# HiKapok/DAN

Hardware: AMD Instinct MI355X
Metric: 640x640 images/sec/node (train fwd+bwd) (higher is better)
Workload: dtype bf16; 1 GPU; S3FD VGG-16 backbone + 6 detection heads, 640x640 bf16 training (fwd+bwd+SGD), batch 16 per GPU; global_batch=16, parallelism=dp1, anchors_per_image=34125, step_launch=eager, rccl_ranks=1, weight_gradient_stream=True

## Files before the change

### dan_amd/_lib.py

```python
import ctypes
import os

import torch

_HERE = os.path.dirname(os.path.abspath(__file__))
ACT_NAME = os.environ.get("DANHIP_DTYPE", "bf16").lower()
if ACT_NAME not in ("bf16", "fp16"):
    raise ValueError("DANHIP_DTYPE must be bf16 or fp16, got %r" % ACT_NAME)
ACT_DTYPE = torch.float16 if ACT_NAME == "fp16" else torch.bfloat16
SO_PATH = os.path.join(_HERE, "libdanhip_f16.so" if ACT_NAME == "fp16" else "libdanhip.so")
if os.environ.get("DANHIP_LIB_PATH"):
    SO_PATH = os.path.abspath(os.environ["DANHIP_LIB_PATH"])

F32, BF16 = 0, 1
SPLIT3 = 3


class ConvDesc(ctypes.Structure):
    _fields_ = [(n, ctypes.c_int32) for n in ("N", "H", "W", "Cin", "Ho", "Wo", "Cout", "kh", "kw", "stride")]


class ConvPitch(ctypes.Structure):
    _fields_ = [(n, ctypes.c_int32) for n in ("x_pitch", "y_pitch", "aux_pitch")]


class PackEntry(ctypes.Structure):
    _fields_ = [("w_hwio", ctypes.c_void_p), ("wf_packed", ctypes.c_void_p), ("wb_packed", ctypes.c_void_p)] + \
               [(n, ctypes.c_int32) for n in ("kh", "kw", "cin", "cin_real", "cout", "rows_f", "cols_f", "rows_b", "cols_b", "co8", "first_block", "pad_")]


HEADS_MAX_LEVELS = 8


class HeadLevel(ctypes.Structure):
    _fields_ = [("h", ctypes.c_void_p), ("dy", ctypes.c_void_p)] + [(n, ctypes.c_int32) for n in ("HW", "Ch", "nneg", "npos", "off", "co_pad")]


class JpegInfo(ctypes.Structure):
    _fields_ = [(n, ctypes.c_int32) for n in ("width", "height", "ncomp", "mode", "reason", "reserved")] + [("coef_count", ctypes.c_int64)]


class JpegDesc(ctypes.Structure):
    _fields_ = [(n, ctypes.c_int32) for n in ("width", "height", "ncomp", "mode")] + \
               [(n, ctypes.c_int32 * 3) for n in ("blocks_w", "blocks_h", "comp_w", "comp_h", "quant_index")] + \
               [(n, ctypes.c_int32) for n in ("status", "idct_groups", "rgb_groups")] + [("reserved", ctypes.c_int32 * 2)] + \
               [("coef_offset", ctypes.c_int64), ("coef_count", ctypes.c_int64), ("plane_offset", ctypes.c_int64 * 3),
                ("out_offset", ctypes.c_int64), ("quant", (ctypes.c_uint16 * 64) * 4)]


P = ctypes.c_void_p
I32 = ctypes.c_int32
I64 = ctypes.c_int64
FL = ctypes.c_float
DESC = ctypes.POINTER(ConvDesc)

SIGNATURES = {
    "danhip_conv_packed_dims": [DESC, ctypes.c_int, ctypes.POINTER(I64), ctypes.POINTER(I64)],
    "danhip_pack_conv_weight": [DESC, P, I32, P, P, P],
    "danhip_conv2d_fwd_pool": [DESC, P, P, P, P, P, P],
    "danhip_pack_entry_init": [ctypes.POINTER(PackEntry), DESC, P, I32, P, P, I32, ctypes.POINTER(ctypes.c_int32)],
    "danhip_pack_conv_weights_batched": [P, I32, I32, P],
    "danhip_conv2d_fwd": [DESC, P, P, P, P, ctypes.c_int, ctypes.c_int, P, P],
    "danhip_conv2d_fwd_ws": [DESC, P, P, P, P, ctypes.c_int, ctypes.c_int, P, P, ctypes.c_size_t, P],
    "danhip_conv2d_fwd_f32": [DESC, P, P, P, P, ctypes.c_int, P, P],
# ... 54 lines not shown
    "danhip_dynamic_anchor_routing_eval": [P, P, P, P, I64, I32, I32, I32, I32, I32, P, P, P, ctypes.c_size_t, P],
    "danhip_dynamic_anchor_routing_train": [P, P, P, P, I64, I32, I32, I32, I32, I32, FL, FL, ctypes.c_uint64, ctypes.c_uint64, P, P, P, P,
                                            ctypes.c_size_t, P],
    "danhip_nms": [P, I32, I32, I32, FL, P, P, P],
    "danhip_argsort_desc_f32": [P, I64, I32, P, P, ctypes.c_size_t, P],
    "danhip_augment_preprocess": [P, I32, I32, I32, ctypes.POINTER(ctypes.c_int32), ctypes.POINTER(ctypes.c_float), I32, I32, I32, I32, I32, P, I32, I32,
                                  P, ctypes.c_size_t, P],
    "danhip_deform_psroi_pool_fwd": [P, P, P, P, P, I32, I32, I32, I32, I32, I32, I32, I32, I32, FL, FL, I32, I32, P],
    "danhip_deform_psroi_pool_bwd": [P, P, P, P, P, P, P, I32, I32, I32, I32, I32, I32, I32, I32, I32, I32, FL, FL, I32, I32, P],
    "danhip_maxpool3x3s2_same_fwd": [P, P, I32, I32, I32, I32, P],
    "danhip_maxpool3x3s2_same_bwd": [P, P, P, I32, I32, I32, I32, P],
    "danhip_resize_u8_linear": [P, I32, I32, P, I32, I32, I32, ctypes.c_double, ctypes.c_double, P],
    "danhip_bbox_vote": [P, P, I32, I32, ctypes.c_double, I32, P, P, P, ctypes.c_size_t, P],
    "danhip_wider_quantize": [P, ctypes.c_int, P, P, I32, I32, I32, P, P, I32, I32, P, P],
    "danhip_wider_score_range": [P, I64, P, P, ctypes.c_size_t, P],
    "danhip_wider_eval": [P, P, I64, P, P, P, I64, P, I32, I32, I32, I32, ctypes.c_double, P, ctypes.c_size_t, P, P],
    "danhip_wider_ap": [P, ctypes.c_size_t, P, I64, I32, I32, I32, P, P, P, P, P, P],
    "danhip_deform_sample_fwd": [P, P, P, I32, I32, I32, I32, I32, I32, I32, I32, I32, P],
    "danhip_deform_sample_bwd": [P, P, P, P, P, I32, I32, I32, I32, I32, I32, I32, I32, I32, ctypes.c_int, P, ctypes.c_size_t, P],
    "danhip_deform_conv_fwd": [P, P, P, P, P, I32, I32, I32, I32, I32, I32, I32, I32, I32, I32, ctypes.c_int, P, ctypes.c_size_t, P],
    "danhip_deform_conv_bwd": [P, P, P, P, P, P, P, P, I32, I32, I32, I32, I32, I32, I32, I32, I32, I32, ctypes.c_int, P, ctypes.c_size_t, P],
    "danhip_deform_conv_bwd_with_col": [P, P, P, P, P, P, P, P, P, I32, I32, I32, I32, I32, I32, I32, I32, I32, I32, ctypes.c_int, P, ctypes.c_size_t, P],
    "danhip_deform_conv_bwd_deliver": [P, P, P, P, P, P, P, P, P, I32, I32, I32, I32, I32, I32, I32, I32, I32, I32, ctypes.c_int, ctypes.c_int, P, ctypes.c_size_t, P],
    "danhip_cast_pad_f32_to_bf16": [P, P, P, I64, I32, I32, P],
    "danhip_head_split_fwd": [P, P, P, I32, I32, I32, I32, I32, I32, I32, P],
    "danhip_head_split_bwd": [P, P, P, P, I32, I32, I32, I32, I32, I32, I32, P],
    "danhip_heads_split_fwd": [ctypes.POINTER(HeadLevel), I32, P, P, I32, I32, P],
    "danhip_heads_grad_pad": [ctypes.POINTER(HeadLevel), I32, P, P, I32, I32, P],
    "danhip_hard_neg_select": [P, P, P, P, P, P, I32, I32, FL, ctypes.c_int, P],
    "danhip_detection_loss_fwd": [P, P, P, P, P, P, P, P, I32, I32, P],
    "danhip_detection_loss_bwd": [P, P, P, P, P, P, P, FL, FL, I32, I32, P],
    "danhip_sgd_momentum_flat": [P, P, P, P, P, P, I32, I64, FL, FL, FL, P, P],
    "danhip_sgd_momentum_flat_dynamic": [P, P, P, P, P, P, I32, I64, FL, FL, P, P, P],
    "danhip_anchors_generate": [P, P, P, P, P, P, I32, I32, I32, FL, FL, FL, I32, P],
    "danhip_iou_matrix": [P, P, P, P, P, P, P, I32, I32, P],
    "danhip_dual_max_match": [P, I32, I32, FL, FL, ctypes.c_int, P, P, P, ctypes.c_size_t, P],
    "danhip_small_mining_match": [P, I32, I32, FL, FL, FL, I32, FL, P, P, P, ctypes.c_size_t, P],
    "danhip_encode_anchors": [P, P, P, P, P, P, P, P, P, I32, FL, FL, FL, FL, FL, P],
    "danhip_decode_anchors": [P, P, P, P, P, P, I32, I32, FL, FL, FL, FL, P],
    "danhip_face_scores": [P, P, P, FL, I64, P],
    "danhip_comm_load": [ctypes.c_char_p],
    "danhip_comm_rccl_version": [ctypes.POINTER(ctypes.c_int)],
    "danhip_comm_unique_id": [P],
    "danhip_comm_create": [P, I32, I32, I32, ctypes.POINTER(ctypes.c_void_p)],
    "danhip_comm_destroy": [P],
    "danhip_comm_info": [P, ctypes.POINTER(I32), ctypes.POINTER(I32), ctypes.POINTER(I32)],
    "danhip_comm_async_error": [P, ctypes.POINTER(I32)],
    "danhip_comm_abort": [P],
    "danhip_comm_allreduce_sum": [P, P, I64, ctypes.c_int, P],
    "danhip_comm_reduce_scatter_sum": [P, P, P, I64, ctypes.c_int, P],
    "danhip_comm_allgather": [P, P, P, I64, ctypes.c_int, P],
    "danhip_jpeg_entropy_decode_batch": [P, P, I32, I32, P, I64, P, P],
    "danhip_jpeg_entropy_decode_batch_ex": [P, P, I32, I32, ctypes.c_uint32, P, I64, P, P],
    "danhip_jpeg_scan_prepare_batch_ex": [P, P, I32, ctypes.c_uint32, P, ctypes.c_size_t, I64, P, P],
    "danhip_jpeg_reconstruct_batch": [P, I64, P, P, I32, P, I64, P, ctypes.c_size_t, P, P],
    "danhip_jpeg_scan_prepare_batch": [P, P, I32, P, ctypes.c_size_t, I64, P, P],
    "danhip_jpeg_huffman_decode_batch": [P, P, ctypes.c_size_t, I32, P, I64, P, P, P, ctypes.c_size_t, P, P, P],
    "danhip_jpeg_entropy_emulate_batch": [P, ctypes.c_size_t, I32, P, P, I64, I32, P, P],
    "danhip_encode_anchors_batched": [P] * 11 + [I32, I32, I32, I32, I32, FL, FL, FL, I32, FL, FL, FL, FL, FL, FL, P, P, P, P, P,
                                                 ctypes.c_size_t, P],
}

_lib = None


class DanhipError(RuntimeError):
# ... 128 lines not shown
```

### dan_amd/csrc/capi.cpp

```cpp
#include <cstdarg>
#include <cstdio>
#include <cstdlib>
#include <cstring>
#include <atomic>
#include <mutex>

#include <hip/hip_runtime.h>

#include "../../include/danhip.h"

static thread_local char g_err[512] = "";

void danhip_set_error(const char* fmt, ...) {
  va_list ap;
  va_start(ap, fmt);
  vsnprintf(g_err, sizeof(g_err), fmt, ap);
  va_end(ap);
}

extern "C" const char* danhip_last_error(void) { return g_err; }
extern "C" int danhip_version(void) { return 10; }
extern "C" int danhip_act_dtype(void) {
#ifdef DANHIP_FP16
  return DANHIP_F16;
#else
  return DANHIP_BF16;
#endif
}

namespace {
struct Opt { const char* name; const char* env; int def; std::atomic<int> value; };
Opt g_opts[] = {{"splitk", "DANHIP_SPLITK", 1, {0}}, {"wgrad_slab", "DANHIP_WGRAD_SLAB", 1, {0}}, {"halo_b2", "DANHIP_HALO_B2", 0, {0}},
                {"wgrad_b2", "DANHIP_WGRAD_B2", 0, {0}}, {"halo_general_epilogue", "DANHIP_HALO_GENERAL_EPILOGUE", 0, {0}},
                {"deform_bwd_form", "DANHIP_DEFORM_BWD_FORM", 0, {0}}, {"pw_dgrad_ld_bn", "DANHIP_PW_DGRAD_LD_BN", 128, {0}},
                {"wgrad_c8", "DANHIP_WGRAD_C8", 1, {0}}, {"deform_dx_untiled", "DANHIP_DEFORM_DX_UNTILED", 0, {0}},
                {"deterministic", "DANHIP_DETERMINISTIC", 0, {0}}};
std::once_flag g_opts_once;
Opt* find_opt(const char* name) {
  std::call_once(g_opts_once, [] {
    for (Opt& o : g_opts) { const char* e = getenv(o.env); o.value.store(e ? atoi(e) : o.def, std::memory_order_relaxed); }
  });
  if (!name) return nullptr;
  for (Opt& o : g_opts)
    if (strcmp(o.name, name) == 0) return &o;
  return nullptr;
}
}

int danhip_option(const char* name) {
  Opt* o = find_opt(name);
  return o ? o->value.load(std::memory_order_relaxed) : 0;
}
extern "C" int danhip_get_option(const char* name) { return danhip_option(name); }

// ... 16 lines not shown
```

### dan_amd/csrc/loss.hip

```cpp
#include "common.h"

namespace {

__device__ __forceinline__ float block_sum(float v, float* sh) {
#pragma unroll
  for (int o = 32; o > 0; o >>= 1) v += __shfl_xor(v, o, 64);
  const int w = threadIdx.x >> 6, nw = blockDim.x >> 6;
  if ((threadIdx.x & 63) == 0) sh[w] = v;
  __syncthreads();
  float t = 0.f;
  for (int i = 0; i < nw; ++i) t += sh[i];
  __syncthreads();
  return t;
}

__global__ void head_split_fwd_kernel(const float* __restrict__ h, float* __restrict__ loc, float* __restrict__ cls, int B, int HW, int Ch,
                                      int nneg, int npos, int A, int off) {
  const long total = (long)B * HW;
  for (long m = (long)blockIdx.x * blockDim.x + threadIdx.x; m < total; m += (long)gridDim.x * blockDim.x) {
    const int b = (int)(m / HW), p = (int)(m % HW);
    const float* r = h + m * Ch;
    const long a = (long)b * A + off + p;
    *reinterpret_cast<float4*>(loc + a * 4) = make_float4(r[0], r[1], r[2], r[3]);
    float ng = r[4];
    for (int i = 1; i < nneg; ++i) ng = fmaxf(ng, r[4 + i]);
    float ps = r[4 + nneg];
    for (int i = 1; i < npos; ++i) ps = fmaxf(ps, r[4 + nneg + i]);
    *reinterpret_cast<float2*>(cls + a * 2) = make_float2(ng, ps);
  }
}

__global__ void head_split_bwd_kernel(const float* __restrict__ h, const float* __restrict__ dloc, const float* __restrict__ dcls,
                                      float* __restrict__ dy, int B, int HW, int Ch, int nneg, int npos, int A, int off) {
// ... 267 lines not shown
    float4 d = make_float4(0.f, 0.f, 0.f, 0.f);
    if (s == 2) {
      const float4 p = *reinterpret_cast<const float4*>(loc + i * 4);
      const float4 t = *reinterpret_cast<const float4*>(loc_t + i * 4);
      const float df[4] = {p.x - t.x, p.y - t.y, p.z - t.z, p.w - t.w};
      float o[4];
#pragma unroll
      for (int j = 0; j < 4; ++j) o[j] = (fabsf(df[j]) < 1.f ? df[j] : (df[j] > 0.f ? 1.f : -1.f)) * kl;
      d = make_float4(o[0], o[1], o[2], o[3]);
    }
    *reinterpret_cast<float4*>(dloc + i * 4) = d;
  }
}

__global__ void sgd_momentum_flat_kernel(float* __restrict__ w, const float* __restrict__ g, float* __restrict__ v, const long* __restrict__ seg,
                                         const float* __restrict__ gmult, const float* __restrict__ wdc, int nseg, long total, float lr,
                                         float momentum, float gscale, float* __restrict__ l2_out, const float* __restrict__ dyn,
                                         float* __restrict__ l2_part) {
  __shared__ float sh[8];
  float l2 = 0.f;
  bool skip = false;
  if (dyn) { gscale = 1.f / dyn[0]; skip = dyn[3] != 0.f; }
  const long n4 = total >> 2;
  const long stride = (long)gridDim.x * blockDim.x;
  long q = (long)blockIdx.x * blockDim.x + threadIdx.x;
  int lo = 0;
  if (q < n4) {
    int hi = nseg;
    while (hi - lo > 1) { const int mid = (lo + hi) >> 1; if (seg[mid] <= q * 4) lo = mid; else hi = mid; }
  }
  auto update = [&](long qq, int sg, float4 wi, const float4 gi, float4 vi) __attribute__((always_inline)) {
    const float c = wdc[sg], gm = gmult[sg];
    l2 += 0.5f * c * (wi.x * wi.x + wi.y * wi.y + wi.z * wi.z + wi.w * wi.w);
    vi.x = momentum * vi.x + (gi.x * gscale + c * wi.x) * gm;
    vi.y = momentum * vi.y + (gi.y * gscale + c * wi.y) * gm;
    vi.z = momentum * vi.z + (gi.z * gscale + c * wi.z) * gm;
    vi.w = momentum * vi.w + (gi.w * gscale + c * wi.w) * gm;
    wi.x -= lr * vi.x; wi.y -= lr * vi.y; wi.z -= lr * vi.z; wi.w -= lr * vi.w;
    if (!skip) {
      reinterpret_cast<float4*>(v)[qq] = vi;
      reinterpret_cast<float4*>(w)[qq] = wi;
    }
  };
  for (; q + stride < n4; q += 2 * stride) {
    const long q1 = q + stride;
    const float4 w0 = reinterpret_cast<const float4*>(w)[q], w1 = reinterpret_cast<const float4*>(w)[q1];
    const float4 g0 = reinterpret_cast<const float4*>(g)[q], g1 = reinterpret_cast<const float4*>(g)[q1];
    const float4 v0 = reinterpret_cast<const float4*>(v)[q], v1 = reinterpret_cast<const float4*>(v)[q1];
    while (lo + 1 < nseg && seg[lo + 1] <= q * 4) ++lo;
    int lo1 = lo;
    while (lo1 + 1 < nseg && seg[lo1 + 1] <= q1 * 4) ++lo1;
    update(q, lo, w0, g0, v0);
    update(q1, lo1, w1, g1, v1);
    lo = lo1;
  }
  for (; q < n4; q += stride) {
    while (lo + 1 < nseg && seg[lo + 1] <= q * 4) ++lo;
    update(q, lo, reinterpret_cast<const float4*>(w)[q], reinterpret_cast<const float4*>(g)[q], reinterpret_cast<const float4*>(v)[q]);
  }
  if (l2_out) {
    l2 = block_sum(l2, sh);
    if (threadIdx.x == 0) {
      if (l2_part) l2_part[blockIdx.x] = l2;
      else atomicAdd(l2_out, l2);
    }
  }
}

__global__ void grad_nonfinite_kernel(const float* __restrict__ g, long total, float* __restrict__ dyn) {
  bool bad = false;
  const long n4 = total >> 2;
// ... 225 lines not shown
```

### dan_amd/ops.py

```python
import contextlib
import ctypes
import os

import torch

from . import _lib
from ._lib import ACT_DTYPE as ACT, BF16, F32, SPLIT3, ConvDesc, call, ptr, stream


class OpsContext(object):
    __slots__ = ("USE_SPLITK", "USE_SLOTS", "USE_RELU_BITS", "USE_POOL_ARG", "USE_JUNCTION", "POOL_ONLY_TRAIN", "KEEP_DEFORM_COL", "WGRAD_STREAM", "WGRAD_FIRST", "FUSE_FIRST_WGRAD", "HEADS_BATCHED", "SPLIT_EVAL", "deterministic", "TRACE",
                 "PROFILE", "PROFILE_BYTES", "GRAD_READY_HOOK", "LOSS_SCALE_DEV", "wgrad")

    def __init__(self, **overrides):
        env = os.environ.get
        self.USE_SPLITK = True
        self.USE_SLOTS = True
        self.USE_RELU_BITS = env("DANHIP_RELU_BITS", "1") == "1"
        self.USE_POOL_ARG = env("DANHIP_POOL_ARG", "1") == "1"
        self.USE_JUNCTION = env("DANHIP_JUNCTION", "1") == "1"
        self.POOL_ONLY_TRAIN = env("DANHIP_POOL_ONLY_TRAIN", "1") == "1"
        self.KEEP_DEFORM_COL = True
        self.WGRAD_STREAM = env("DANHIP_WGRAD_STREAM", "1") == "1"
        self.WGRAD_FIRST = env("DANHIP_WGRAD_FIRST", "0") == "1"
        self.FUSE_FIRST_WGRAD = env("DANHIP_FUSE_FIRST_WGRAD", "1") == "1"
        self.HEADS_BATCHED = env("DANHIP_HEADS_BATCHED", "1") == "1"
        self.SPLIT_EVAL = False
        self.deterministic = env("DANHIP_DETERMINISTIC", "0") == "1"
        self.TRACE = self.PROFILE = self.PROFILE_BYTES = None
        self.GRAD_READY_HOOK = self.LOSS_SCALE_DEV = None
        self.wgrad = {"on": False, "side": None, "main": None, "keep": []}
        for k, v in overrides.items():
            setattr(self, k, v)


_CTX = OpsContext()
_CTX_FIELDS = frozenset(OpsContext.__slots__) - {"wgrad"}


def context():
    return _CTX


@contextlib.contextmanager
def use_context(ctx):
    global _CTX
    prev, _CTX = _CTX, ctx
    _sync_deterministic(prev, ctx)
    try:
        yield ctx
    finally:
        _CTX = prev
        _sync_deterministic(ctx, prev)


def _sync_deterministic(old, new):
    if bool(old.deterministic) != bool(new.deterministic):
        call("danhip_set_option", b"deterministic", 1 if new.deterministic else 0)

# ... 74 lines not shown
    st = _stamp(w_param)
    if e.stamp != st:
        wd = w_param.detach()
        if not (wd.dtype == torch.float32 and wd.is_contiguous()):
            raise RuntimeError("packed_weights: a kernel variable of shape %s arrives as a non-contiguous view (strides %s): it is a member of a "
                               "fused parameter block, which only the fused op consumes - set the fused / unfused switches BEFORE the "
                               "trainer (FlatParams) is built, not between calls" % (tuple(wd.shape), tuple(wd.stride())))
        call("danhip_pack_conv_weight", ctypes.byref(e.d), ptr(wd), wd.shape[2], ptr(e.wf), ptr(e.wb), stream())
        e.stamp = st
    return e.wf, (e.wb if need_bwd else None)


def repack_all(key=None, select=None):
    entries = [(e, e.ref()) for e in _PACKED.values()]
    entries = [(e, p) for e, p in entries if p is not None and (select is None or select(p))]
    if not entries:
        return
    tabs = _PACK_TABLE_OF
    tab = tabs.get(key)
    ids, ptrs = [id(p) for _, p in entries], [p.data_ptr() for _, p in entries]
    if tab is None or tab[3] != ids or tab[4] != ptrs:
        arr = (_lib.PackEntry * len(entries))()
        first = 0
        nb = ctypes.c_int32()
        for i, (e, p) in enumerate(entries):
            call("danhip_pack_entry_init", ctypes.byref(arr[i]), ctypes.byref(e.d), ptr(p.detach()), p.shape[2], ptr(e.wf), ptr(e.wb), first,
                 ctypes.byref(nb))
            first += nb.value
        host = torch.frombuffer(bytearray(bytes(arr)), dtype=torch.uint8)
        tab = tabs[key] = (len(entries), host.to(entries[0][1].device), first, ids, ptrs)
    n, dev_tab, blocks, _, _ = tab
    call("danhip_pack_conv_weights_batched", ptr(dev_tab), n, blocks, stream())
    for e, p in entries:
        e.stamp = _stamp(p)


def _grad_sink(p):
    return getattr(p, "_danhip_grad", None)


def _sink_trainable(t):
    ms = getattr(t, "_danhip_members", None)
    return ms is not None and any(m.requires_grad for m in ms)


def _prof_begin(st=None):
    if _CTX.PROFILE is None:
        return None
    e = torch.cuda.Event(enable_timing=True)
    e.record(st if st is not None else torch.cuda.current_stream())
    return e


def _prof_end(e0, d, which, st=None, wrote_y=True, pooled=False):
    if e0 is None:
        return
    e1 = torch.cuda.Event(enable_timing=True)
    e1.record(st if st is not None else torch.cuda.current_stream())
    if which == 2:
        label = _lib.lib().danhip_conv_wgrad_kernel_label(ctypes.byref(d)).decode()
    else:
        label = _lib.lib().danhip_conv_kernel_label(ctypes.byref(d), which).decode()
    cin = d.Cin
    flops = 2.0 * d.N * d.Ho * d.Wo * cin * d.Cout * d.kh * d.kw
    _CTX.PROFILE.setdefault(label, []).append((e0, e1, flops))
    if _CTX.PROFILE_BYTES is not None:
# ... 1603 lines not shown
```

### dan_amd/trainer.py

```python
import atexit
import ctypes
import os
import sys
import weakref

import torch
import torch.distributed as dist

from ._lib import call, ptr, stream


def comm_timeout_s():
    return float(os.environ.get("DANHIP_COMM_TIMEOUT_S", "300"))


DEADLINE_EXIT_CODE = 75


def _die(msg):
    sys.stderr.write("dan_amd: FATAL (rank %s): %s\n" % (os.environ.get("RANK", "0"), msg))
    sys.stderr.flush()
    os._exit(DEADLINE_EXIT_CODE)


# ... 374 lines not shown
            self.g.index_fill_(0, self.struct_zero_idx, 0.0)

    def range_plan(self, s, e):
        k0, k1 = self.starts.index(s), (self.starts.index(e) if e < self.total else len(self.starts))
        rel = (self.seg[k0:k1 + 1] - s).contiguous()
        idx = None
        if self.struct_zero_idx is not None:
            m = (self.struct_zero_idx >= s) & (self.struct_zero_idx < e)
            idx = self.struct_zero_idx[m].contiguous() if bool(m.any()) else None
        return k0, k1 - k0, rel, idx

    def sgd_range(self, s, e, plan, lr, momentum=0.9, grad_scale=1.0):
        k0, nseg, rel, idx = plan
        if idx is not None:
            self.g.index_fill_(0, idx, 0.0)
        off = ctypes.c_void_p
        base = lambda t, elems: off(t.data_ptr() + 4 * elems)
        call("danhip_sgd_momentum_flat", base(self.w, s), base(self.g, s), base(self.v, s), ptr(rel), base(self.gmult, k0), base(self.wdc, k0), nseg,
             e - s, float(lr), float(momentum), float(grad_scale), ptr(self.l2), stream())

    def sgd_step(self, lr, momentum=0.9, grad_scale=1.0, dynamic_state=None, deterministic=False):
        self.mask_structured()
        self.l2.zero_()
        if dynamic_state is not None:
            call("danhip_sgd_momentum_flat_dynamic", ptr(self.w), ptr(self.g), ptr(self.v), ptr(self.seg), ptr(self.gmult), ptr(self.wdc),
                 len(self.names), self.total, float(lr), float(momentum), ptr(dynamic_state), ptr(self.l2), stream())
        elif deterministic:
            if getattr(self, "_sgd_ws", None) is None:
                from . import _lib
                self._sgd_ws = torch.empty(int(_lib.lib().danhip_sgd_workspace_bytes()), dtype=torch.uint8, device=self.w.device)
            call("danhip_sgd_momentum_flat_ws", ptr(self.w), ptr(self.g), ptr(self.v), ptr(self.seg), ptr(self.gmult), ptr(self.wdc), len(self.names),
                 self.total, float(lr), float(momentum), float(grad_scale), ptr(self.l2), ptr(self._sgd_ws), self._sgd_ws.numel(), stream())
        else:
            call("danhip_sgd_momentum_flat", ptr(self.w), ptr(self.g), ptr(self.v), ptr(self.seg), ptr(self.gmult), ptr(self.wdc), len(self.names),
                 self.total, float(lr), float(momentum), float(grad_scale), ptr(self.l2), stream())
        from . import ops
        ops.WEIGHT_EPOCH += 1
        ops.repack_all()


class GradBuckets(object):

    def __init__(self, flat, bucket_bytes=32 << 20, tail_bytes=2 << 20):
        self.flat = flat
        self.on_bucket = None
        self.local = False
        self.enabled = (dist.is_available() and dist.is_initialized() and dist.get_world_size() > 1) or (os.environ.get("DANHIP_FORCE_DIST") == "1" and flat.g.is_cuda)
        self.fake = (not self.enabled) and os.environ.get("DANHIP_FAKE_ALLREDUCE") == "1" and flat.g.is_cuda
        self.enabled = self.enabled or self.fake
        self.bucket_bytes = bucket_bytes
        per = max(1, bucket_bytes // 4)
        self.bounds = []
        end = flat.total
        cur_end = end
        for s in reversed(flat.starts):
            if cur_end - s >= per:
                self.bounds.append((s, cur_end))
                cur_end = s
        if cur_end > 0:
            self.bounds.append((0, cur_end))
        s0, e0 = self.bounds[-1]
        tail = max(1, tail_bytes // 4)
        if e0 - s0 > 2 * tail:
            cut = max((st for st in flat.starts if s0 < st <= s0 + tail), default=None)
            if cut is not None and cut < e0:
                self.bounds[-1:] = [(cut, e0), (s0, cut)]
# ... 181 lines not shown
```

### include/danhip.h

```cpp
#ifndef DANHIP_H_
#define DANHIP_H_
#include <stddef.h>
#include <stdint.h>

#ifdef __cplusplus
extern "C" {
#endif

#define DANHIP_OK 0
#define DANHIP_EINVAL (-1)
#define DANHIP_ELAUNCH (-2)
#define DANHIP_EWORKSPACE (-3)

#define DANHIP_F32 0
#define DANHIP_BF16 1
#define DANHIP_F16 2
#define DANHIP_SPLIT3 3

const char* danhip_last_error(void);
int danhip_version(void);
int danhip_set_option(const char* name, int value);
int danhip_get_option(const char* name);
int danhip_act_dtype(void);

// ... 129 lines not shown
int danhip_head_split_bwd(const float* h, const float* dloc, const float* dcls, float* dy, int32_t B, int32_t HW, int32_t Ch,
                          int32_t nneg, int32_t npos, int32_t A, int32_t anchor_offset, void* stream);
#define DANHIP_HEADS_MAX_LEVELS 8
typedef struct danhip_head_level {
  const float* h;
  uint16_t* dy;
  int32_t HW, Ch, nneg, npos;
  int32_t off;
  int32_t co_pad;
} danhip_head_level;
int danhip_heads_split_fwd(const danhip_head_level* levels, int32_t nlevels, float* loc, float* cls, int32_t B, int32_t A, void* stream);
int danhip_heads_grad_pad(const danhip_head_level* levels, int32_t nlevels, const float* dloc, const float* dcls, int32_t B, int32_t A,
                          void* stream);
int danhip_hard_neg_select(const float* cls, const int32_t* labels, float* score, int32_t* counts, float* thr, int32_t* k_out,
                           int32_t B, int32_t A, float negative_ratio, int at_least_one, void* stream);
int danhip_detection_loss_fwd(const float* cls, const float* loc, const int32_t* labels, const float* loc_targets,
                              const float* score, const float* thr, uint8_t* sel, float* acc4, int32_t B, int32_t A,
                              void* stream);
int danhip_detection_loss_fwd_ws(const float* cls, const float* loc, const int32_t* labels, const float* loc_targets,
                                 const float* score, const float* thr, uint8_t* sel, float* acc4, int32_t B, int32_t A,
                                 void* ws, size_t ws_bytes, void* stream);
int danhip_detection_loss_bwd(const float* cls, const float* loc, const float* loc_targets, const uint8_t* sel,
                              const float* acc4, float* dcls, float* dloc, float ce_scale, float loc_scale, int32_t B,
                              int32_t A, void* stream);
int danhip_sgd_momentum_flat(float* w, const float* g, float* v, const int64_t* seg_starts, const float* gmult,
                             const float* wd_coef, int32_t nseg, int64_t total, float lr, float momentum, float grad_scale,
                             float* l2_out, void* stream);
int danhip_sgd_momentum_flat_ws(float* w, const float* g, float* v, const int64_t* seg_starts, const float* gmult,
                                const float* wd_coef, int32_t nseg, int64_t total, float lr, float momentum, float grad_scale,
                                float* l2_out, void* ws, size_t ws_bytes, void* stream);
int danhip_sgd_momentum_flat_dynamic(float* w, const float* g, float* v, const int64_t* seg_starts, const float* gmult,
                                     const float* wd_coef, int32_t nseg, int64_t total, float lr, float momentum,
                                     float* loss_scale_state, float* l2_out, void* stream);

int danhip_anchors_generate(float* ymin, float* xmin, float* ymax, float* xmax, const float* anchor_h, const float* anchor_w,
                            int32_t depth, int32_t layer_h, int32_t layer_w, float stride, float offset_h, float offset_w,
                            int32_t out_offset, void* stream);
int danhip_iou_matrix(const float* ymin, const float* xmin, const float* ymax, const float* xmax, const uint8_t* inside_mask,
                      const float* gt_boxes, float* overlaps, int32_t A, int32_t G, void* stream);
size_t danhip_match_workspace_bytes(int32_t A, int32_t G);
int danhip_dual_max_match(const float* overlaps, int32_t A, int32_t G, float low_thres, float high_thres, int ignore_between,
                          int32_t* match_indices, float* match_scores, void* workspace, size_t workspace_bytes, void* stream);
int danhip_small_mining_match(const float* overlaps, int32_t A, int32_t G, float negative_low_thres, float negative_high_thres,
                              float positive_thres, int32_t min_match, float stop_positive_thres, int32_t* match_indices,
                              float* match_scores, void* workspace, size_t workspace_bytes, void* stream);
int danhip_encode_anchors(const float* ymin, const float* xmin, const float* ymax, const float* xmax, const float* gt_boxes,
                          const int32_t* match_indices, float* targets, int32_t* labels, float* matched_gt, int32_t A,
                          float ps0, float ps1, float ps2, float ps3, float scale, void* stream);
size_t danhip_encode_anchors_batched_workspace_bytes(int32_t B, int32_t A, int32_t total_gt);
int danhip_encode_anchors_batched(const float* ymin, const float* xmin, const float* ymax, const float* xmax, const float* match_ymin,
                                  const float* match_xmin, const float* match_ymax, const float* match_xmax, const uint8_t* inside_mask,
                                  const float* gt_boxes, const int32_t* gt_offsets, int32_t B, int32_t A, int32_t total_gt, int32_t max_gt,
                                  int32_t match_mining, float negative_low_thres, float ignore_thres, float positive_thres,
                                  int32_t min_match, float stop_positive_thres, float ps0, float ps1, float ps2, float ps3, float scale,
                                  float* targets, int32_t* labels, float* scores, float* matched_gt, void* workspace,
                                  size_t workspace_bytes, void* stream);
int danhip_decode_anchors(const float* pred, const float* ymin, const float* xmin, const float* ymax, const float* xmax,
                          float* boxes, int32_t B, int32_t A, float ps0, float ps1, float ps2, float ps3, void* stream);

int danhip_face_scores(const float* cls, float* score, int32_t* mask, float threshold, int64_t n, void* stream);


int danhip_deform_sample_fwd(const uint16_t* x, const uint16_t* offsets, uint16_t* S, int32_t N, int32_t H, int32_t W, int32_t C,
                             int32_t kh, int32_t kw, int32_t stride, int32_t dilation, int32_t deformable_group, void* stream);
size_t danhip_deform_sample_bwd_workspace_bytes(int32_t N, int32_t H, int32_t W, int32_t C);
int danhip_deform_sample_bwd(const uint16_t* x, const uint16_t* offsets, const uint16_t* dS, uint16_t* dx, uint16_t* d_offsets,
// ... 199 lines not shown
```

Before: 1319 images/sec.

## Fuse SGD momentum update with bf16 conv weight repacking into one kernel

Adds a kernel that applies the SGD momentum update and, for conv weights, writes the updated values straight into the bf16 forward and backward packed layouts through a shared-memory transpose tile. Residual parameter ranges are covered by a flat float4 path in the same launch. This removes the separate repack launch and the re-read of fp32 weights the next step would otherwise need. The SGD arithmetic is moved into a shared helper with explicit fma, which can change rounding slightly. The per-tile path uses scalar strided loads instead of float4, and the plan is cached on the host.

```diff
diff --git a/dan_amd/_lib.py b/dan_amd/_lib.py
--- a/dan_amd/_lib.py
+++ b/dan_amd/_lib.py
@@ -30,6 +30,7 @@
 
 
 HEADS_MAX_LEVELS = 8
+SGD_PACK_RANGE_BLOCKS = 1024
 
 
 class HeadLevel(ctypes.Structure):
@@ -150,6 +151,7 @@
     "danhip_detection_loss_bwd": [P, P, P, P, P, P, P, FL, FL, I32, I32, P],
     "danhip_sgd_momentum_flat": [P, P, P, P, P, P, I32, I64, FL, FL, FL, P, P],
     "danhip_sgd_momentum_flat_dynamic": [P, P, P, P, P, P, I32, I64, FL, FL, P, P, P],
+    "danhip_sgd_momentum_pack": [P, P, P, P, P, P, I32, I64, FL, FL, FL, P, P, P, I32, P, P, I32, I32, P],
     "danhip_anchors_generate": [P, P, P, P, P, P, I32, I32, I32, FL, FL, FL, I32, P],
     "danhip_iou_matrix": [P, P, P, P, P, P, P, I32, I32, P],
     "danhip_dual_max_match": [P, I32, I32, FL, FL, ctypes.c_int, P, P, P, ctypes.c_size_t, P],
diff --git a/dan_amd/csrc/capi.cpp b/dan_amd/csrc/capi.cpp
--- a/dan_amd/csrc/capi.cpp
+++ b/dan_amd/csrc/capi.cpp
@@ -19,7 +19,7 @@
 }
 
 extern "C" const char* danhip_last_error(void) { return g_err; }
-extern "C" int danhip_version(void) { return 10; }
+extern "C" int danhip_version(void) { return 11; }
 extern "C" int danhip_act_dtype(void) {
 #ifdef DANHIP_FP16
   return DANHIP_F16;
diff --git a/dan_amd/csrc/loss.hip b/dan_amd/csrc/loss.hip
--- a/dan_amd/csrc/loss.hip
+++ b/dan_amd/csrc/loss.hip
@@ -1,4 +1,5 @@
 #include "common.h"
+#include "sgd_update.h"
 
 namespace {
 
@@ -332,11 +333,10 @@
   auto update = [&](long qq, int sg, float4 wi, const float4 gi, float4 vi) __attribute__((always_inline)) {
     const float c = wdc[sg], gm = gmult[sg];
     l2 += 0.5f * c * (wi.x * wi.x + wi.y * wi.y + wi.z * wi.z + wi.w * wi.w);
-    vi.x = momentum * vi.x + (gi.x * gscale + c * wi.x) * gm;
-    vi.y = momentum * vi.y + (gi.y * gscale + c * wi.y) * gm;
-    vi.z = momentum * vi.z + (gi.z * gscale + c * wi.z) * gm;
-    vi.w = momentum * vi.w + (gi.w * gscale + c * wi.w) * gm;
-    wi.x -= lr * vi.x; wi.y -= lr * vi.y; wi.z -= lr * vi.z; wi.w -= lr * vi.w;
+    dh_sgd_update(wi.x, gi.x, vi.x, c, gm, momentum, gscale, lr);
+    dh_sgd_update(wi.y, gi.y, vi.y, c, gm, momentum, gscale, lr);
+    dh_sgd_update(wi.z, gi.z, vi.z, c, gm, momentum, gscale, lr);
+    dh_sgd_update(wi.w, gi.w, vi.w, c, gm, momentum, gscale, lr);
     if (!skip) {
       reinterpret_cast<float4*>(v)[qq] = vi;
       reinterpret_cast<float4*>(w)[qq] = wi;
diff --git a/dan_amd/csrc/sgd_pack.hip b/dan_amd/csrc/sgd_pack.hip
--- /dev/null
+++ b/dan_amd/csrc/sgd_pack.hip
@@ -0,0 +1,281 @@
+#include "common.h"
+#include "sgd_update.h"
+
+namespace {
+
+__device__ __forceinline__ float block_sum256(float v, float* sh) {
+#pragma unroll
+  for (int o = 32; o > 0; o >>= 1) v += __shfl_xor(v, o, 64);
+  if ((threadIdx.x & 63) == 0) sh[threadIdx.x >> 6] = v;
+  __syncthreads();
+  return (sh[0] + sh[1]) + (sh[2] + sh[3]);
+}
+
+struct SgdPackArgs {
+  float* w;
+  float* g;
+  float* v;
+  const long* seg;
+  const float* gmult;
+  const float* wdc;
+  int nseg;
+  float lr, momentum, gscale;
+  float* l2_out;
+  const danhip_pack_entry* tab;
+  int n, tile_blocks;
+  const long* ranges;
+  int nranges, zero_grad;
+};
+
+__device__ __forceinline__ int seg_of(const long* __restrict__ seg, int nseg, long i) {
+  int lo = 0, hi = nseg;
+  while (hi - lo > 1) { const int mid = (lo + hi) >> 1; if (seg[mid] <= i) lo = mid; else hi = mid; }
+  return lo;
+}
+
+__device__ __forceinline__ void tile_block(const SgdPackArgs& a, float (*tile)[33], float* sh) {
+  int lo = 0, hi = a.n - 1;
+  while (lo < hi) {
+    const int mid = (lo + hi + 1) >> 1;
+    if (a.tab[mid].first_block <= (int)blockIdx.x) lo = mid; else hi = mid - 1;
+  }
+  const danhip_pack_entry e = a.tab[lo];
+  const int lb = (int)blockIdx.x - e.first_block;
+  const long off = e.w_hwio - a.w;
+  const int sg = seg_of(a.seg, a.nseg, off);
+  const float c = a.wdc[sg], gm = a.gmult[sg];
+  float* __restrict__ w = a.w + off;
+  float* __restrict__ g = a.g + off;
+  float* __restrict__ v = a.v + off;
+  const int taps = e.kh * e.kw;
+  const int tid = threadIdx.x;
+  const int ctiles = (e.rows_f + 31) / 32;
+  const int tco = lb % ctiles, tk = lb / ctiles;
+  const int co0 = tco * 32, k0 = tk * 64;
+  const int tx = tid & 31, ty = tid >> 5;
+  long idx[8];
+  float wi[8], gi[8], vi[8];
+#pragma unroll
+  for (int r = 0; r < 8; ++r) {
+    const int k = k0 + ty + 8 * r;
+    const int tap = k / e.cin, ch = k - tap * e.cin;
+    idx[r] = (co0 + tx < e.cout && tap < taps && ch < e.cin_real) ? ((long)tap * e.cin_real + ch) * e.cout + co0 + tx : -1;
+    wi[r] = gi[r] = vi[r] = 0.f;
+    if (idx[r] >= 0) { wi[r] = w[idx[r]]; gi[r] = g[idx[r]]; vi[r] = v[idx[r]]; }
+  }
+  float l2 = 0.f;
+#pragma unroll
+  for (int r = 0; r < 8; ++r) {
+    float wn = 0.f;
+    if (idx[r] >= 0) {
+      l2 += wi[r] * wi[r];
+      wn = wi[r];
+      float vn = vi[r];
+      dh_sgd_update(wn, gi[r], vn, c, gm, a.momentum, a.gscale, a.lr);
+      v[idx[r]] = vn;
+      w[idx[r]] = wn;
+      if (a.zero_grad) g[idx[r]] = 0.f;
+    }
+    tile[ty + 8 * r][tx] = wn;
+  }
+  __syncthreads();
+  {
+    bf16_t* __restrict__ wf = e.wf_packed;
+    const int col = tid >> 3, kq = tid & 7;
+    const int kg = k0 + kq * 8;
+    const int tap = kg / e.cin, c0 = kg - tap * e.cin;
+    if (co0 + col < e.cout && tap < taps && c0 < e.cin_real) {
+      bf16_t* dst = wf + (long)(co0 + col) * e.cols_f + kg;
+      if (c0 + 8 <= e.cin_real) {
+        uint4 o;
+        o.x = pack2bf(tile[kq * 8 + 0][col], tile[kq * 8 + 1][col]);
+        o.y = pack2bf(tile[kq * 8 + 2][col], tile[kq * 8 + 3][col]);
+        o.z = pack2bf(tile[kq * 8 + 4][col], tile[kq * 8 + 5][col]);
+        o.w = pack2bf(tile[kq * 8 + 6][col], tile[kq * 8 + 7][col]);
+        *reinterpret_cast<uint4*>(dst) = o;
+      } else {
+        for (int i = 0; c0 + i < e.cin_real; ++i) dst[i] = f2bf(tile[kq * 8 + i][col]);
+      }
+    }
+  }
+  if (e.wb_packed) {
+    bf16_t* __restrict__ wb = e.wb_packed;
+    const int kl = tid >> 2, j = tid & 3;
+    const int k = k0 + kl;
+    const int tap = k / e.cin, ch = k - tap * e.cin;
+    const int cf = co0 + 8 * j;
+    if (tap < taps && ch < e.cin_real && cf < e.cout) {
+      const int fi = tap / e.kw, fj = tap - fi * e.kw;
+      const int tapf = (e.kh - 1 - fi) * e.kw + (e.kw - 1 - fj);
+      bf16_t* dst = wb + (long)ch * e.cols_b + tapf * e.co8 + cf;
+      if (cf + 8 <= e.cout) {
+        uint4 o;
+        o.x = pack2bf(tile[kl][8 * j + 0], tile[kl][8 * j + 1]);
+        o.y = pack2bf(tile[kl][8 * j + 2], tile[kl][8 * j + 3]);
+        o.z = pack2bf(tile[kl][8 * j + 4], tile[kl][8 * j + 5]);
+        o.w = pack2bf(tile[kl][8 * j + 6], tile[kl][8 * j + 7]);
+        *reinterpret_cast<uint4*>(dst) = o;
+      } else {
+        for (int i = 0; cf + i < e.cout; ++i) dst[i] = f2bf(tile[kl][8 * j + i]);
+      }
+    }
+  }
+  if (a.l2_out) {
+    l2 = block_sum256(0.5f * c * l2, sh);
+    if (tid == 0) atomicAdd(a.l2_out, l2);
+  }
+}
+
+__device__ __forceinline__ void range_block(const SgdPackArgs& a, float* sh) {
+  const int rb = (int)blockIdx.x - a.tile_blocks;
+  int lo = 0, hi = a.nranges - 1;
+  while (lo < hi) {
+    const int mid = (lo + hi + 1) >> 1;
+    if (a.ranges[3 * mid + 2] <= rb) lo = mid; else hi = mid - 1;
+  }
+  const long s = a.ranges[3 * lo], e = a.ranges[3 * lo + 1];
+  const int first = (int)a.ranges[3 * lo + 2];
+  const int nb = (lo + 1 < a.nranges ? (int)a.ranges[3 * lo + 5] : (int)gridDim.x - a.tile_blocks) - first;
+  const int lb = rb - first;
+  float* __restrict__ w = a.w;
+  float* __restrict__ g = a.g;
+  float* __restrict__ v = a.v;
+  const long* __restrict__ seg = a.seg;
+  const int nseg = a.nseg;
+  float l2 = 0.f;
+  const long s4 = (s + 3) & ~3l;
+  if (lb == 0 && s + (long)threadIdx.x < (s4 < e ? s4 : e)) {
+    const long i = s + threadIdx.x;
+    const int sg = seg_of(seg, nseg, i);
+    const float c = a.wdc[sg];
+    float wn = w[i], vn = v[i];
+    l2 += 0.5f * c * (wn * wn);
+    dh_sgd_update(wn, g[i], vn, c, a.gmult[sg], a.momentum, a.gscale, a.lr);
+    v[i] = vn;
+    w[i] = wn;
+    if (a.zero_grad) g[i] = 0.f;
+  }
+  const long q_end = e >> 2;
+  const long stride = (long)nb * 256;
+  long q = (s4 >> 2) + (long)lb * 256 + threadIdx.x;
+  int sl = 0;
+  if (q < q_end) sl = seg_of(seg, nseg, q * 4);
+  auto update = [&](long qq, int sg, float4 wi, const float4 gi, float4 vi) __attribute__((always_inline)) {
+    const float c = a.wdc[sg], gm = a.gmult[sg];
+    l2 += 0.5f * c * (wi.x * wi.x + wi.y * wi.y + wi.z * wi.z + wi.w * wi.w);
+    dh_sgd_update(wi.x, gi.x, vi.x, c, gm, a.momentum, a.gscale, a.lr);
+    dh_sgd_update(wi.y, gi.y, vi.y, c, gm, a.momentum, a.gscale, a.lr);
+    dh_sgd_update(wi.z, gi.z, vi.z, c, gm, a.momentum, a.gscale, a.lr);
+    dh_sgd_update(wi.w, gi.w, vi.w, c, gm, a.momentum, a.gscale, a.lr);
+    reinterpret_cast<float4*>(v)[qq] = vi;
+    reinterpret_cast<float4*>(w)[qq] = wi;
+    if (a.zero_grad) reinterpret_cast<float4*>(g)[qq] = make_float4(0.f, 0.f, 0.f, 0.f);
+  };
+  for (; q + stride < q_end; q += 2 * stride) {
+    const long q1 = q + stride;
+    const float4 w0 = reinterpret_cast<const float4*>(w)[q], w1 = reinterpret_cast<const float4*>(w)[q1];
+    const float4 g0 = reinterpret_cast<const float4*>(g)[q], g1 = reinterpret_cast<const float4*>(g)[q1];
+    const float4 v0 = reinterpret_cast<const float4*>(v)[q], v1 = reinterpret_cast<const float4*>(v)[q1];
+    while (sl + 1 < nseg && seg[sl + 1] <= q * 4) ++sl;
+    int sl1 = sl;
+    while (sl1 + 1 < nseg && seg[sl1 + 1] <= q1 * 4) ++sl1;
+    update(q, sl, w0, g0, v0);
+    update(q1, sl1, w1, g1, v1);
+    sl = sl1;
+  }
+  for (; q < q_end; q += stride) {
+    while (sl + 1 < nseg && seg[sl + 1] <= q * 4) ++sl;
+    update(q, sl, reinterpret_cast<const float4*>(w)[q], reinterpret_cast<const float4*>(g)[q], reinterpret_cast<const float4*>(v)[q]);
+  }
+  if (a.l2_out) {
+    l2 = block_sum256(l2, sh);
+    if (threadIdx.x == 0) atomicAdd(a.l2_out, l2);
+  }
+}
+
+__global__ __launch_bounds__(256) void sgd_momentum_pack_kernel(const SgdPackArgs a) {
+  __shared__ float tile[64][33];
+  __shared__ float sh[4];
+  if ((int)blockIdx.x < a.tile_blocks) tile_block(a, tile, sh);
+  else range_block(a, sh);
+}
+
+inline int round_up8(int v) { return (v + 7) / 8 * 8; }
+
+inline long range_blocks(long s, long e) {
+  long b = ((e - s + 3) / 4 + 255) / 256;
+  if (b > DANHIP_SGD_PACK_RANGE_BLOCKS) b = DANHIP_SGD_PACK_RANGE_BLOCKS;
+  return b < 1 ? 1 : b;
+}
+
+}
+
+extern "C" int danhip_sgd_momentum_pack(float* w, float* g, float* v, const int64_t* seg_starts, const float* gmult, const float* wd_coef,
+                                        int32_t nseg, int64_t total, float lr, float momentum, float grad_scale, float* l2_out,
+                                        const danhip_pack_entry* entries_host, const danhip_pack_entry* entries_dev, int32_t n_entries,
+                                        const int64_t* ranges_host, const int64_t* ranges_dev, int32_t n_ranges, int32_t zero_grad,
+                                        void* stream) {
+  DH_REQUIRE(w && g && v && seg_starts && gmult && wd_coef && nseg > 0 && total > 0, DANHIP_EINVAL, "sgd_momentum_pack: bad arguments");
+  DH_REQUIRE(total % 4 == 0 && (((uintptr_t)w | (uintptr_t)g | (uintptr_t)v) & 15) == 0, DANHIP_EINVAL,
+             "sgd_momentum_pack: buffers must be 16-byte aligned, total a multiple of 4");
+  DH_REQUIRE(n_entries >= 0 && n_ranges >= 0 && n_entries + n_ranges > 0, DANHIP_EINVAL, "sgd_momentum_pack: empty plan");
+  DH_REQUIRE((n_entries == 0 || (entries_host && entries_dev)) && (n_ranges == 0 || (ranges_host && ranges_dev)), DANHIP_EINVAL,
+             "sgd_momentum_pack: null table");
+  DH_REQUIRE(!(l2_out && danhip_option("deterministic") != 0), DANHIP_EINVAL,
+             "sgd_momentum_pack: l2_out has no deterministic form (call danhip_sgd_momentum_flat_ws and danhip_pack_conv_weights_batched)");
+  long tiles = 0, rblocks = 0, covered = 0, pos = 0;
+  int ie = 0, ir = 0;
+  while (ie < n_entries || ir < n_ranges) {
+    long es = -1, rs = -1;
+    if (ie < n_entries) {
+      const danhip_pack_entry& e = entries_host[ie];
+      DH_REQUIRE(e.w_hwio && e.wf_packed, DANHIP_EINVAL, "sgd_momentum_pack: entry %d: null pointer", ie);
+      DH_REQUIRE(e.kh > 0 && e.kw > 0 && e.cin > 0 && e.cin % 8 == 0 && e.cin_real > 0 && e.cin_real <= e.cin && e.cout > 0 && e.rows_f >= e.cout &&
+                 e.cols_f >= e.kh * e.kw * e.cin && e.cols_f % 64 == 0 && e.co8 == round_up8(e.cout), DANHIP_EINVAL,
+                 "sgd_momentum_pack: entry %d: inconsistent dimensions (fill it with danhip_pack_entry_init)", ie);
+      DH_REQUIRE((long)e.rows_f * e.cols_f < (1ll << 31) && (!e.wb_packed || (long)e.rows_b * e.cols_b < (1ll << 31)), DANHIP_EINVAL,
+                 "sgd_momentum_pack: entry %d: packed matrix exceeds 2^31 elements", ie);
+      DH_REQUIRE(!e.wb_packed || (e.rows_b >= e.cin_real && e.cols_b >= e.kh * e.kw * e.co8), DANHIP_EINVAL,
+                 "sgd_momentum_pack: entry %d: inconsistent backward dimensions", ie);
+      DH_REQUIRE(e.pad_ == ((e.rows_f + 31) / 32) * (e.cols_f / 64) && e.first_block == tiles, DANHIP_EINVAL,
+                 "sgd_momentum_pack: entry %d: first_block must be the running sum of the forward tiles (pad_)", ie);
+      DH_REQUIRE(e.w_hwio >= w && e.w_hwio < w + total, DANHIP_EINVAL, "sgd_momentum_pack: entry %d lies outside the flat buffer", ie);
+      es = e.w_hwio - w;
+    }
+    if (ir < n_ranges) {
+      rs = ranges_host[3 * ir];
+      DH_REQUIRE(rs >= 0 && ranges_host[3 * ir + 1] > rs && ranges_host[3 * ir + 1] <= total && ranges_host[3 * ir + 1] % 4 == 0, DANHIP_EINVAL,
+                 "sgd_momentum_pack: range %d: need 0 <= start < end <= total, end a multiple of 4", ir);
+      DH_REQUIRE(ranges_host[3 * ir + 2] == rblocks, DANHIP_EINVAL,
+                 "sgd_momentum_pack: range %d: first workgroup must be the running sum of min(%d, ceil(ceil(length / 4) / 256))", ir,
+                 DANHIP_SGD_PACK_RANGE_BLOCKS);
+    }
+    const bool take_entry = es >= 0 && (rs < 0 || es < rs);
+    const long s = take_entry ? es : rs;
+    DH_REQUIRE(s >= pos, DANHIP_EINVAL, "sgd_momentum_pack: %s %d overlaps its predecessor or is out of order", take_entry ? "entry" : "range",
+               take_entry ? ie : ir);
+    if (take_entry) {
+      const danhip_pack_entry& e = entries_host[ie];
+      const long numel = (long)e.kh * e.kw * e.cin_real * e.cout;
+      DH_REQUIRE(s + numel <= total, DANHIP_EINVAL, "sgd_momentum_pack: entry %d ends outside the flat buffer", ie);
+      pos = s + numel; covered += numel; tiles += e.pad_;
+      DH_REQUIRE(tiles < (1l << 30) - 8192, DANHIP_EINVAL, "sgd_momentum_pack: too many tiles");
+      ++ie;
+    } else {
+      const long e = ranges_host[3 * ir + 1];
+      pos = e; covered += e - s; rblocks += range_blocks(s, e);
+      ++ir;
+    }
+  }
+  DH_REQUIRE(covered == total, DANHIP_EINVAL, "sgd_momentum_pack: the plan covers %ld of %ld elements (every float exactly once)", covered,
+             (long)total);
+  SgdPackArgs a;
+  a.w = w; a.g = g; a.v = v;
+  a.seg = reinterpret_cast<const long*>(seg_starts); a.gmult = gmult; a.wdc = wd_coef; a.nseg = nseg;
+  a.lr = lr; a.momentum = momentum; a.gscale = grad_scale; a.l2_out = l2_out;
+  a.tab = entries_dev; a.n = n_entries; a.tile_blocks = (int)tiles;
+  a.ranges = reinterpret_cast<const long*>(ranges_dev); a.nranges = n_ranges; a.zero_grad = zero_grad != 0;
+  hipLaunchKernelGGL(sgd_momentum_pack_kernel, dim3((unsigned)(tiles + rblocks)), dim3(256), 0, (hipStream_t)stream, a);
+  DH_LAUNCH_CHECK();
+  return DANHIP_OK;
+}
diff --git a/dan_amd/csrc/sgd_update.h b/dan_amd/csrc/sgd_update.h
--- /dev/null
+++ b/dan_amd/csrc/sgd_update.h
@@ -0,0 +1,8 @@
+#pragma once
+#include <hip/hip_runtime.h>
+
+__device__ __forceinline__ void dh_sgd_update(float& w, float g, float& v, float c, float gm, float momentum, float gscale, float lr) {
+  const float d = __fmaf_rn(g, gscale, __fmul_rn(c, w));
+  v = __fmaf_rn(momentum, v, __fmul_rn(d, gm));
+  w = __fmaf_rn(-lr, v, w);
+}
diff --git a/dan_amd/ops.py b/dan_amd/ops.py
--- a/dan_amd/ops.py
+++ b/dan_amd/ops.py
@@ -9,7 +9,7 @@
 
 
 class OpsContext(object):
-    __slots__ = ("USE_SPLITK", "USE_SLOTS", "USE_RELU_BITS", "USE_POOL_ARG", "USE_JUNCTION", "POOL_ONLY_TRAIN", "KEEP_DEFORM_COL", "WGRAD_STREAM", "WGRAD_FIRST", "FUSE_FIRST_WGRAD", "HEADS_BATCHED", "SPLIT_EVAL", "deterministic", "TRACE",
+    __slots__ = ("USE_SPLITK", "USE_SLOTS", "USE_RELU_BITS", "USE_POOL_ARG", "USE_JUNCTION", "POOL_ONLY_TRAIN", "KEEP_DEFORM_COL", "WGRAD_STREAM", "WGRAD_FIRST", "FUSE_FIRST_WGRAD", "HEADS_BATCHED", "FUSED_UPDATE", "SPLIT_EVAL", "deterministic", "TRACE",
                  "PROFILE", "PROFILE_BYTES", "GRAD_READY_HOOK", "LOSS_SCALE_DEV", "wgrad")
 
     def __init__(self, **overrides):
@@ -25,6 +25,7 @@
         self.WGRAD_FIRST = env("DANHIP_WGRAD_FIRST", "0") == "1"
         self.FUSE_FIRST_WGRAD = env("DANHIP_FUSE_FIRST_WGRAD", "1") == "1"
         self.HEADS_BATCHED = env("DANHIP_HEADS_BATCHED", "1") == "1"
+        self.FUSED_UPDATE = env("DANHIP_FUSED_UPDATE", "1") == "1"
         self.SPLIT_EVAL = False
         self.deterministic = env("DANHIP_DETERMINISTIC", "0") == "1"
         self.TRACE = self.PROFILE = self.PROFILE_BYTES = None
@@ -165,6 +166,81 @@
     n, dev_tab, blocks, _, _ = tab
     call("danhip_pack_conv_weights_batched", ptr(dev_tab), n, blocks, stream())
     for e, p in entries:
+        e.stamp = _stamp(p)
+
+
+class FusedUpdatePlanError(ValueError):
+    """The cached packings and the flat buffer do not form a plan danhip_sgd_momentum_pack can run: the caller takes the two launches."""
+
+
+def fused_update_plan(spans, starts, total, range_blocks=_lib.SGD_PACK_RANGE_BLOCKS):
+    import bisect
+    if total <= 0 or total % 4 or not starts or starts[0] != 0 or any(b <= a for a, b in zip(starts, starts[1:])) or starts[-1] >= total:
+        raise FusedUpdatePlanError("segment table does not describe a buffer of %d floats" % total)
+    order = sorted(range(len(spans)), key=lambda i: spans[i][0])
+    ranges, pos, first = [], 0, 0
+
+    def residual(s, e):
+        nonlocal first
+        ranges.append((s, e, first))
+        first += max(1, min(range_blocks, -(-(-(-(e - s) // 4)) // 256)))
+    for i in order:
+        off, n = spans[i]
+        if n <= 0 or off < 0 or off + n > total:
+            raise FusedUpdatePlanError("span %d [%d, %d) lies outside the buffer" % (i, off, off + n))
+        if off < pos:
+            raise FusedUpdatePlanError("span %d [%d, %d) overlaps its predecessor" % (i, off, off + n))
+        if off % 4:
+            raise FusedUpdatePlanError("span %d begins at %d: not a float4 boundary" % (i, off))
+        k = bisect.bisect_right(starts, off) - 1
+        if off + n > (starts[k + 1] if k + 1 < len(starts) else total):
+            raise FusedUpdatePlanError("span %d [%d, %d) straddles the segment boundary %d" % (i, off, off + n, starts[k + 1]))
+        if off > pos:
+            residual(pos, off)
+        pos = off + n
+    if pos < total:
+        residual(pos, total)
+    return order, ranges
+
+
+def fused_update_table(flat):
+    w0, total = flat.w.data_ptr(), flat.total
+    entries = [(e, e.ref()) for e in _PACKED.values()]
+    entries = [(e, p) for e, p in entries if p is not None and w0 <= p.data_ptr() < w0 + 4 * total]
+    key = ("fused", id(flat))
+    ids, ptrs = [id(p) for _, p in entries], [p.data_ptr() for _, p in entries] + [w0]
+    tab = _PACK_TABLE_OF.get(key)
+    if tab is not None and tab[0] == ids and tab[1] == ptrs:
+        return tab[2]
+    plan = None
+    try:
+        if not entries:
+            raise FusedUpdatePlanError("no cached packing lies in this buffer")
+        for _, p in entries:
+            if not (p.dtype == torch.float32 and p.is_contiguous()):
+                raise FusedUpdatePlanError("a cached packing belongs to a non-contiguous view")
+        order, ranges = fused_update_plan([((p.data_ptr() - w0) // 4, p.numel()) for _, p in entries], list(flat.starts), total)
+        entries = [entries[i] for i in order]
+        if any(e.stamp is None for e, _ in entries):
+            repack_all()
+        arr = (_lib.PackEntry * len(entries))()
+        first, nb = 0, ctypes.c_int32()
+        for i, (e, p) in enumerate(entries):
+            call("danhip_pack_entry_init", ctypes.byref(arr[i]), ctypes.byref(e.d), ptr(p.detach()), p.shape[2], ptr(e.wf), ptr(e.wb), first,
+                 ctypes.byref(nb))
+            first += arr[i].pad_
+        host_r = torch.tensor(ranges, dtype=torch.int64).reshape(-1, 3)
+        dev = flat.w.device
+        plan = (arr, torch.frombuffer(bytearray(bytes(arr)), dtype=torch.uint8).to(dev), len(entries), host_r, host_r.to(dev), len(ranges),
+                entries)
+    except FusedUpdatePlanError:
+        plan = None
+    _PACK_TABLE_OF[key] = (ids, ptrs, plan)
+    return plan
+
+
+def fused_update_done(plan):
+    for e, p in plan[6]:
         e.stamp = _stamp(p)
 
 
diff --git a/dan_amd/trainer.py b/dan_amd/trainer.py
--- a/dan_amd/trainer.py
+++ b/dan_amd/trainer.py
@@ -430,6 +430,16 @@
             call("danhip_sgd_momentum_flat_ws", ptr(self.w), ptr(self.g), ptr(self.v), ptr(self.seg), ptr(self.gmult), ptr(self.wdc), len(self.names),
                  self.total, float(lr), float(momentum), float(grad_scale), ptr(self.l2), ptr(self._sgd_ws), self._sgd_ws.numel(), stream())
         else:
+            from . import ops
+            plan = ops.fused_update_table(self) if (ops.context().FUSED_UPDATE and self.w.is_cuda) else None
+            if plan is not None:
+                arr, dev_tab, n, host_r, dev_r, nr, _ = plan
+                call("danhip_sgd_momentum_pack", ptr(self.w), ptr(self.g), ptr(self.v), ptr(self.seg), ptr(self.gmult), ptr(self.wdc),
+                     len(self.names), self.total, float(lr), float(momentum), float(grad_scale), ptr(self.l2), ctypes.cast(arr, ctypes.c_void_p),
+                     ptr(dev_tab), n, ptr(host_r) if nr else None, ptr(dev_r) if nr else None, nr, 0, stream())
+                ops.WEIGHT_EPOCH += 1
+                ops.fused_update_done(plan)
+                return
             call("danhip_sgd_momentum_flat", ptr(self.w), ptr(self.g), ptr(self.v), ptr(self.seg), ptr(self.gmult), ptr(self.wdc), len(self.names),
                  self.total, float(lr), float(momentum), float(grad_scale), ptr(self.l2), stream())
         from . import ops
diff --git a/include/danhip.h b/include/danhip.h
--- a/include/danhip.h
+++ b/include/danhip.h
@@ -185,6 +185,12 @@
 int danhip_sgd_momentum_flat_dynamic(float* w, const float* g, float* v, const int64_t* seg_starts, const float* gmult,
                                      const float* wd_coef, int32_t nseg, int64_t total, float lr, float momentum,
                                      float* loss_scale_state, float* l2_out, void* stream);
+
+#define DANHIP_SGD_PACK_RANGE_BLOCKS 1024
+int danhip_sgd_momentum_pack(float* w, float* g, float* v, const int64_t* seg_starts, const float* gmult, const float* wd_coef,
+                             int32_t nseg, int64_t total, float lr, float momentum, float grad_scale, float* l2_out,
+                             const danhip_pack_entry* entries_host, const danhip_pack_entry* entries_dev, int32_t n_entries,
+                             const int64_t* ranges_host, const int64_t* ranges_dev, int32_t n_ranges, int32_t zero_grad, void* stream);
 
 int danhip_anchors_generate(float* ymin, float* xmin, float* ymax, float* xmax, const float* anchor_h, const float* anchor_w,
                             int32_t depth, int32_t layer_h, int32_t layer_w, float stride, float offset_h, float offset_w,
```

Measured after the change: 1310 images/sec. No clear change (-0.7%).
